# hku-mars/FAST_LIO

Measured on NVIDIA H100. Metric: scans/sec (30k-pt scan, 1M-pt map iEKF), higher is better.
Workload: dtype f32 geometry / f64 filter

## Files before the change

fast_lio_b200/csrc/filter.cu:

```cuda
#include <dlfcn.h>

#include <algorithm>
#include <chrono>
#include <cstdlib>

#include <cub/device/device_select.cuh>

#include "filter.h"
#include "gj.cuh"
#include "measure.cuh"

namespace fl {

constexpr int PSTRIDE = 96;
constexpr size_t P2P_MAIL_BYTES = sizeof(unsigned long long) * 2 * 2 * P2P_MAX_RANKS * PSTRIDE;
constexpr int SEARCH_THREADS = 256;
constexpr int SEARCH_C_THREADS = 256;
constexpr int RESID_THREADS = 256;
constexpr int MAX_LOGS = 16;

__device__ __forceinline__ void pdl_wait() { asm volatile("griddepcontrol.wait;" ::: "memory"); }
__device__ __forceinline__ void pdl_launch() { asm volatile("griddepcontrol.launch_dependents;" ::: "memory"); }

__device__ __forceinline__ int tri12(int a, int b) { return a * 12 - (a * (a - 1)) / 2 + (b - a); }
// ... 775 lines not shown
                                                                  const double* __restrict__ P, StateIn s) {
    pdl_launch();
    const int b = (int)blockIdx.x;
    state_in(ctl + b, pub + (size_t)b * BATCH_PUB_WORDS, x26 + (size_t)b * XLEN, P + (size_t)b * NDOF * NDOF, s);
}

__global__ void k_count_in(const int* __restrict__ n, int n_max, int* __restrict__ bind) {
    bind[0] = min(max(*n, 0), n_max);
    bind[1] = BIND_SCAN;
}

__device__ __forceinline__ void state_out(const FilterCtl* __restrict__ ctl, double* __restrict__ x26, double* __restrict__ P,
                                          int* __restrict__ status2) {
    const int t = threadIdx.x;
    const int e = ctl->error;
    if (e == 0) {
        for (int i = t; i < NDOF * NDOF; i += STATE_THREADS) P[i] = ctl->P[i];
        if (t < XLEN) x26[t] = ctl->x[t];
    }
    if (t == 0) { status2[0] = e == 0 ? FL_OK : (e == 2 ? FL_ERR_NCCL : FL_ERR_STATE); status2[1] = ctl->n_pass; }
}
__global__ void __launch_bounds__(STATE_THREADS) k_state_out(const FilterCtl* __restrict__ ctl, double* __restrict__ x26,
                                                             double* __restrict__ P, int* __restrict__ status2) {
    state_out(ctl, x26, P, status2);
}
__global__ void __launch_bounds__(STATE_THREADS) k_batch_state_out(const FilterCtl* __restrict__ ctl, double* __restrict__ x26,
                                                                   double* __restrict__ P, int* __restrict__ status2) {
    const int b = (int)blockIdx.x;
    state_out(ctl + b, x26 + (size_t)b * XLEN, P + (size_t)b * NDOF * NDOF, status2 + 2 * b);
}

__global__ void k_flags_clear(unsigned char* __restrict__ flag_add, unsigned char* __restrict__ flag_no, const int* __restrict__ n, int n_max) {
    const int q = blockIdx.x * blockDim.x + threadIdx.x;
    if (q < n_max && q >= *n) { flag_add[q] = 0; flag_no[q] = 0; }
}

struct NcclUniqueId { char internal[128]; };
struct NcclApi {
    void* lib = nullptr;
    int (*GetUniqueId)(NcclUniqueId*) = nullptr;
    int (*CommInitRank)(void**, int, NcclUniqueId, int) = nullptr;
    int (*AllReduce)(const void*, void*, size_t, int, int, void*, cudaStream_t) = nullptr;
    int (*CommDestroy)(void*) = nullptr;
    const char* (*GetErrorString)(int) = nullptr;
};
static NcclApi* load_nccl() {
    static NcclApi api;
    if (api.lib) return &api;
    const char* names[] = {"libnccl.so.2", "libnccl.so"};
    for (const char* nm : names) { api.lib = dlopen(nm, RTLD_NOW | RTLD_GLOBAL); if (api.lib) break; }
    if (!api.lib) { set_last_error("NCCL: cannot dlopen libnccl.so.2: %s", dlerror()); return nullptr; }
    api.GetUniqueId = (int (*)(NcclUniqueId*))dlsym(api.lib, "ncclGetUniqueId");
    api.CommInitRank = (int (*)(void**, int, NcclUniqueId, int))dlsym(api.lib, "ncclCommInitRank");
    api.AllReduce = (int (*)(const void*, void*, size_t, int, int, void*, cudaStream_t))dlsym(api.lib, "ncclAllReduce");
    api.CommDestroy = (int (*)(void*))dlsym(api.lib, "ncclCommDestroy");
    api.GetErrorString = (const char* (*)(int))dlsym(api.lib, "ncclGetErrorString");
    if (!api.GetUniqueId || !api.CommInitRank || !api.AllReduce || !api.CommDestroy) {
        set_last_error("NCCL: missing symbols in libnccl");
        api.lib = nullptr;
        return nullptr;
    }
    return &api;
}
int nccl_unique_id(void* out128) {
    NcclApi* api = load_nccl();
    if (!api) return FL_ERR_NCCL;
    NcclUniqueId id;
    int rc = api->GetUniqueId(&id);
    if (rc != 0) { set_last_error("ncclGetUniqueId failed: %d", rc); return FL_ERR_NCCL; }
    memcpy(out128, &id, 128);
    return FL_OK;
}

Filter::Filter(Map* map, int max_points) : map_(map), max_points_(max_points) {
    memset(&scan_, 0, sizeof(scan_));
    for (int i = 0; i < NDOF; i++) limit_[i] = 0.001;
}
Filter::~Filter() {
    cudaSetDevice(map_->device());
    if (comm_ && nccl_) nccl_->CommDestroy(comm_);
    for (int r = 0; r < P2P_MAX_RANKS; r++) if (peer_ptr_[r]) cudaIpcCloseMemHandle(peer_ptr_[r]);
    mailbox_.release(); p2p_.release();
    body_.release(); nearest_.release(); nearest_cnt_.release(); selected_.release(); normvec_.release(); plane_.release(); srange_.release();
    partials_.release(); red_.release(); ctl_.release(); ctl0_.release(); logs_.release(); pub_.release();
    mi_world_.release(); mi_flag_add_.release(); mi_flag_no_.release(); mi_list_add_.release(); mi_list_no_.release(); mi_tmp_.release(); mi_counts_.release();
    d_bind_.release();
    b_body_.release(); b_ctl_.release(); b_pub_.release(); b_partials_.release();
    b_nearest_.release(); b_nearest_cnt_.release(); b_selected_.release(); b_plane_.release(); b_srange_.release();
    if (h_ctl_) cudaFreeHost(h_ctl_);
    if (ev0_) cudaEventDestroy(ev0_);
    if (ev1_) cudaEventDestroy(ev1_);
}

int Filter::init() {
    FL_CUDA(cudaSetDevice(map_->device()));
    if (const char* e = getenv("FASTLIO_B200_NO_PDL")) pdl_ = !(e[0] == '1');
    if (const char* e = getenv("FASTLIO_B200_NO_MIRROR")) mirror_ = !(e[0] == '1');
    if (const char* e = getenv("FASTLIO_B200_SEARCH")) search_mode_ = atoi(e) ? 1 : 0;
    FL_CHECK(ctl_.reserve(sizeof(FilterCtl)));
    FL_CHECK(ctl0_.reserve(sizeof(FilterCtl)));
    FL_CHECK(red_.reserve(sizeof(double) * PSTRIDE));
    FL_CHECK(logs_.reserve(sizeof(PassLog) * MAX_LOGS));
    FL_CHECK(pub_.reserve(512));
    FL_CUDA(cudaMemsetAsync(pub_.ptr, 0, 512, stream()));
    FL_CUDA(cudaMallocHost(&h_ctl_, sizeof(FilterCtl)));
    memset(h_ctl_, 0, sizeof(FilterCtl));
    FL_CUDA(cudaMemsetAsync(ctl_.ptr, 0, sizeof(FilterCtl), stream()));
    FL_CUDA(cudaMemsetAsync(ctl0_.ptr, 0, sizeof(FilterCtl), stream()));
    FL_CUDA(cudaMemsetAsync(logs_.ptr, 0, sizeof(PassLog) * MAX_LOGS, stream()));
    int dev = map_->device(), occ = 0;
    FL_CUDA(cudaDeviceGetAttribute(&sms_, cudaDevAttrMultiProcessorCount, dev));
    if (const char* e = getenv("FASTLIO_B200_SEARCH_OCC")) search_occ_ = atoi(e);
    if (search_occ_ == 6) FL_CUDA(cudaOccupancyMaxActiveBlocksPerMultiprocessor(&occ, k_search<6>, SEARCH_THREADS, 0));
    else if (search_occ_ == 5) FL_CUDA(cudaOccupancyMaxActiveBlocksPerMultiprocessor(&occ, k_search<5>, SEARCH_THREADS, 0));
    else FL_CUDA(cudaOccupancyMaxActiveBlocksPerMultiprocessor(&occ, k_search<4>, SEARCH_THREADS, 0));
    search_grid_max_ = sms_ * std::max(1, occ);
    if (const char* e = getenv("FASTLIO_B200_LEGACY")) fused_ = !(e[0] == '1');
    FL_CUDA(cudaOccupancyMaxActiveBlocksPerMultiprocessor(&occ, k_update<false, 1>, UPD_THREADS, 0));
    upd_capacity_[0][0] = sms_ * std::max(1, occ);
    FL_CUDA(cudaOccupancyMaxActiveBlocksPerMultiprocessor(&occ, k_update<true, 1>, UPD_THREADS, 0));
    upd_capacity_[1][0] = sms_ * std::max(1, occ);
    FL_CUDA(cudaOccupancyMaxActiveBlocksPerMultiprocessor(&occ, k_update<false, 2>, 2 * UPD_THREADS, 0));
    upd_capacity_[0][1] = sms_ * occ;
    FL_CUDA(cudaOccupancyMaxActiveBlocksPerMultiprocessor(&occ, k_update<true, 2>, 2 * UPD_THREADS, 0));
    upd_capacity_[1][1] = sms_ * occ;
    FL_CUDA(cudaOccupancyMaxActiveBlocksPerMultiprocessor(&occ, k_update_n<false, 1>, UPD_THREADS, 0));
    upd_n_capacity_[0][0] = std::min(upd_capacity_[0][0], sms_ * std::max(1, occ));
    FL_CUDA(cudaOccupancyMaxActiveBlocksPerMultiprocessor(&occ, k_update_n<true, 1>, UPD_THREADS, 0));
    upd_n_capacity_[1][0] = std::min(upd_capacity_[1][0], sms_ * std::max(1, occ));
    FL_CUDA(cudaOccupancyMaxActiveBlocksPerMultiprocessor(&occ, k_update_n<false, 2>, 2 * UPD_THREADS, 0));
    upd_n_capacity_[0][1] = std::min(upd_capacity_[0][1], sms_ * occ);
    FL_CUDA(cudaOccupancyMaxActiveBlocksPerMultiprocessor(&occ, k_update_n<true, 2>, 2 * UPD_THREADS, 0));
    upd_n_capacity_[1][1] = std::min(upd_capacity_[1][1], sms_ * occ);
    FL_CUDA(cudaOccupancyMaxActiveBlocksPerMultiprocessor(&occ, k_update_batch<false>, UPD_THREADS, 0));
    batch_cap_[0] = sms_ * occ;
    FL_CUDA(cudaOccupancyMaxActiveBlocksPerMultiprocessor(&occ, k_update_batch<true>, UPD_THREADS, 0));
    batch_cap_[1] = sms_ * occ;
    FL_CHECK(d_bind_.reserve(2 * sizeof(int)));
    FL_CUDA(cudaMemsetAsync(d_bind_.ptr, 0, 2 * sizeof(int), stream()));
    FL_CHECK(partials_.reserve(sizeof(double) * PSTRIDE * (size_t)std::max(upd_capacity_[0][0], upd_capacity_[1][0])));
    max_resid_grid_ = sms_;
    FL_CHECK(partials_.reserve(sizeof(double) * PSTRIDE * (size_t)max_resid_grid_));
    FL_CHECK(reserve(std::max(1, max_points_)));
    return FL_OK;
}

int Filter::reserve(int nq) {
    FL_CHECK(body_.reserve(sizeof(float4) * (size_t)nq));
    FL_CHECK(nearest_.reserve(sizeof(float4) * KNN_K * (size_t)nq));
    { const size_t had = nearest_cnt_.bytes; FL_CHECK(nearest_cnt_.reserve(sizeof(int) * (size_t)nq)); if (nearest_cnt_.bytes != had) FL_CUDA(cudaMemsetAsync(nearest_cnt_.ptr, 0, nearest_cnt_.bytes, stream())); }
    FL_CHECK(selected_.reserve((size_t)nq));
    FL_CHECK(normvec_.reserve(sizeof(float4) * (size_t)nq));
    scan_.nearest = nearest_.as<float4>();
    scan_.nearest_cnt = nearest_cnt_.as<int>();
    scan_.selected = selected_.as<unsigned char>();
    scan_.normvec = normvec_.as<float4>();
    FL_CHECK(plane_.reserve(sizeof(float4) * (size_t)nq));
    scan_.plane = plane_.as<float4>();
    FL_CHECK(srange_.reserve(sizeof(double) * (size_t)nq));
    scan_.srange = srange_.as<double>();
    FL_CHECK(mi_world_.reserve(sizeof(float4) * (size_t)nq));
    FL_CHECK(mi_flag_add_.reserve((size_t)nq));
    FL_CHECK(mi_flag_no_.reserve((size_t)nq));
    FL_CHECK(mi_list_add_.reserve(sizeof(float4) * (size_t)nq));
    FL_CHECK(mi_list_no_.reserve(sizeof(float4) * (size_t)nq));
    FL_CHECK(mi_counts_.reserve(sizeof(int) * 2));
    size_t tmp = 0;
    FL_CUDA(cub::DeviceSelect::Flagged(nullptr, tmp, (const float4*)nullptr, (const unsigned char*)nullptr, (float4*)nullptr, (int*)nullptr, nq));
    FL_CHECK(mi_tmp_.reserve(tmp));
    return FL_OK;
}

int Filter::set_params(int max_iter, const double* limit23, int extrinsic_est_en) {
    if (max_iter < 1 || max_iter + 1 > MAX_LOGS) { set_last_error("set_params: max_iter must be in [1, %d]", MAX_LOGS - 1); return FL_ERR_ARG; }
    max_iter_ = max_iter;
    if (limit23) for (int i = 0; i < NDOF; i++) limit_[i] = limit23[i];
    extrinsic_est_ = extrinsic_est_en ? 1 : 0;
    return FL_OK;
}

int Filter::set_scan_device(const float4* d_body, int nq) {
    FL_CHECK(bind_scan(d_body, nq));
    if (stream_bound_) FL_CUDA(cudaMemsetAsync(d_bind_.as<int>() + 1, 0, sizeof(int), stream()));
    return FL_OK;
}
int Filter::bind_scan(const float4* d_body, int nq) {
    if (nq < 0) { set_last_error("scan: nq < 0"); return FL_ERR_ARG; }
    FL_CUDA(cudaSetDevice(map_->device()));
    FL_CHECK(reserve(std::max(1, nq)));
    scan_.body = d_body;
    scan_.Q = nq;
    if (!shard_set_) { scan_.q_begin = 0; scan_.q_end = nq; }
    dev_count_ = false;
    return FL_OK;
}

int Filter::upload_scan(const float* body_xyzi, int nq) {
    if (nq < 0 || (nq > 0 && !body_xyzi)) { set_last_error("scan: bad arguments"); return FL_ERR_ARG; }
    FL_CUDA(cudaSetDevice(map_->device()));
    FL_CHECK(reserve(std::max(1, nq)));
    if (nq > 0) FL_CUDA(cudaMemcpyAsync(body_.ptr, body_xyzi, sizeof(float4) * (size_t)nq, cudaMemcpyHostToDevice, stream()));
    return set_scan_device(body_.as<float4>(), nq);
}

int Filter::set_shard(int q_begin, int q_end) {
    if (q_begin < 0 || q_end < q_begin) { set_last_error("set_shard: bad range"); return FL_ERR_ARG; }
    scan_.q_begin = q_begin; scan_.q_end = q_end;
    shard_set_ = true;
    return FL_OK;
}

int Filter::upload_state(const double* x26, const double* P, double R, bool snapshot) {
    FL_CUDA(cudaSetDevice(map_->device()));
    FL_CUDA(cudaStreamSynchronize(stream()));
    FilterCtl& c = *h_ctl_;
    c.iter = -1; c.t = 0; c.converge = 1; c.done = 0; c.n_pass = 0; c.error = 0; c.ticket = 0; c.gen = 0;
    c.max_iter = max_iter_;
    c.host_mirror = (mirror_ && !snapshot) ? h_ctl_ : nullptr;
    c.extrinsic_est = extrinsic_est_;
    c.R = R;
    for (int i = 0; i < NDOF; i++) c.limit[i] = limit_[i];
    memcpy(c.x, x26, sizeof(double) * XLEN);
    memcpy(c.x_prop, x26, sizeof(double) * XLEN);
    memcpy(c.P, P, sizeof(double) * NDOF * NDOF);
    memcpy(c.P_prop, P, sizeof(double) * NDOF * NDOF);
    FL_CUDA(cudaMemcpyAsync(ctl_.ptr, h_ctl_, sizeof(FilterCtl), cudaMemcpyHostToDevice, stream()));
    if (snapshot) FL_CUDA(cudaMemcpyAsync(ctl0_.ptr, ctl_.ptr, sizeof(FilterCtl), cudaMemcpyDeviceToDevice, stream()));
    return FL_OK;
}

int Filter::restore_state() {
    FL_CUDA(cudaSetDevice(map_->device()));
    FL_CUDA(cudaMemcpyAsync(ctl_.ptr, ctl0_.ptr, sizeof(FilterCtl), cudaMemcpyDeviceToDevice, stream()));
    return FL_OK;
}

template <class... KArgs, class... Args>
static cudaError_t launch_pdl(void (*kernel)(KArgs...), dim3 grid, int block, cudaStream_t st, bool pdl, Args... args) {
    cudaLaunchConfig_t cfg;
    memset(&cfg, 0, sizeof(cfg));
    cfg.gridDim = grid; cfg.blockDim = dim3((unsigned)block); cfg.dynamicSmemBytes = 0; cfg.stream = st;
    cudaLaunchAttribute attr[1];
    attr[0].id = cudaLaunchAttributeProgrammaticStreamSerialization;
    attr[0].val.programmaticStreamSerializationAllowed = pdl ? 1 : 0;
    cfg.attrs = attr; cfg.numAttrs = 1;
    return cudaLaunchKernelEx(&cfg, kernel, KArgs(args)...);
}

int Filter::complete_neighbours() {
    if (neighbours_complete_ || (scan_.q_begin <= 0 && scan_.q_end >= scan_.Q)) { neighbours_complete_ = true; return FL_OK; }
    FL_CUDA(cudaSetDevice(map_->device()));
    const int keep_b = scan_.q_begin, keep_e = scan_.q_end;
    const int ranges[2][2] = {{0, keep_b}, {keep_e, scan_.Q}};
    for (int r = 0; r < 2; r++) {
        if (ranges[r][1] <= ranges[r][0]) continue;
        scan_.q_begin = ranges[r][0]; scan_.q_end = ranges[r][1];
        UpdArgs a;
        a.m = map_->view();
        if (search_mode_ == 0) a.m.dir.cap = 0;
        a.sc = scan_; a.ctl = ctl_.as<FilterCtl>(); a.partials = partials_.as<double>(); a.red_g = red_.as<double>();
        a.logs = logs_.as<PassLog>(); a.p2p = p2p_.as<P2PState>();
        a.mode = 0; a.max_passes = 1; a.search_only = 1; a.dbg = 0; a.pose_from_search = 1;
        a.pub = pub_.as<unsigned long long>(); a.nonce = ++launch_nonce_;
        const int cap = upd_capacity_[extrinsic_est_ ? 1 : 0][0];
        const int nq = scan_.q_end - scan_.q_begin;
        const int workers = std::max(1, std::min(cap - 1, (nq + UPD_THREADS - 1) / UPD_THREADS));
        cudaError_t e = launch_upd(workers, false, a, upd_pair(nq));
        if (e != cudaSuccess) { scan_.q_begin = keep_b; scan_.q_end = keep_e; set_last_error("complete_neighbours: %s", cudaGetErrorString(e)); return FL_ERR_CUDA; }
    }
    scan_.q_begin = keep_b; scan_.q_end = keep_e;
    neighbours_complete_ = true;
    return FL_OK;
}

int Filter::run_passes() {
    FL_CUDA(cudaSetDevice(map_->device()));
    if (scan_.q_end > scan_.Q) { set_last_error("shard exceeds the scan"); return FL_ERR_ARG; }
    neighbours_complete_ = false;
    launches_ = 0;
    if (fused()) {
        cudaStream_t st = stream();
        if (nranks_ > 1 && !p2p_on_) {
            for (int pass = 0; pass <= max_iter_; pass++) {
                FL_CHECK(launch_update(1, 1, 0));
                int rc = nccl_->AllReduce(red_.ptr, red_.ptr, NRED,  8,  0, comm_, st);
                if (rc != 0) { set_last_error("ncclAllReduce failed: %d", rc); return FL_ERR_NCCL; }
                FL_CHECK(launch_update(1, 3, 0));
                launches_ += 2;
            }
        } else {
            FL_CHECK(launch_update(max_iter_ + 1, nranks_ > 1 ? 2 : 0, 0));
            launches_ = 1;
        }
        FL_CUDA(cudaGetLastError());
        return FL_OK;
    }
    for (int pass = 0; pass <= max_iter_; pass++) {
        FL_CHECK(launch_search_only());
        FL_CHECK(launch_residual_only());
        launches_ += 2;
        if (nranks_ > 1 && !p2p_on_) {
            cudaStream_t st = stream();
            int rc = nccl_->AllReduce(red_.ptr, red_.ptr, NRED,  8,  0, comm_, st);
            if (rc != 0) { set_last_error("ncclAllReduce failed: %d", rc); return FL_ERR_NCCL; }
            FilterCtl* c = ctl_.as<FilterCtl>(); double* rg = red_.as<double>(); PassLog* lg = logs_.as<PassLog>();
            if (extrinsic_est_) { if (solver_) k_solve_only<true, 1><<<1, RESID_THREADS, 0, st>>>(c, rg, scan_, lg); else k_solve_only<true, 0><<<1, RESID_THREADS, 0, st>>>(c, rg, scan_, lg); }
            else { if (solver_) k_solve_only<false, 1><<<1, RESID_THREADS, 0, st>>>(c, rg, scan_, lg); else k_solve_only<false, 0><<<1, RESID_THREADS, 0, st>>>(c, rg, scan_, lg); }
            launches_++;
        }
    }
    FL_CUDA(cudaGetLastError());
    return FL_OK;
}

UpdArgs Filter::upd_args(int max_passes, int mode, int search_only) {
    UpdArgs a;
    a.m = map_->view();
    if (search_mode_ == 0) a.m.dir.cap = 0;
    a.sc = scan_; a.ctl = ctl_.as<FilterCtl>(); a.partials = partials_.as<double>(); a.red_g = red_.as<double>();
    a.logs = logs_.as<PassLog>(); a.p2p = p2p_.as<P2PState>();
    a.mode = mode; a.max_passes = max_passes; a.search_only = search_only;
    a.pub = pub_.as<unsigned long long>(); a.nonce = ++launch_nonce_;
    { const char* e = getenv("FASTLIO_B200_DBG"); a.dbg = e ? atoi(e) : 0; }
    a.pose_from_search = 0;
    return a;
}

int Filter::launch_update(int max_passes, int mode, int search_only, cudaStream_t st) {
    FL_CUDA(cudaSetDevice(map_->device()));
    const int nq = scan_.q_end - scan_.q_begin;
    const UpdArgs a = upd_args(max_passes, mode, search_only);
    const int cap = upd_capacity_[extrinsic_est_ ? 1 : 0][0];
    int workers = mode == 3 ? 0 : std::min(cap - 1, (nq + UPD_THREADS - 1) / UPD_THREADS);
    if (workers < 0) workers = 0;
    FL_CUDA(launch_upd(workers, pdl_, a, upd_pair(nq), st));
    return FL_OK;
}

int Filter::upd_pair(int nq) const {
    if (const char* e = getenv("FASTLIO_B200_PAIR")) if (e[0] == '1') return 1;
    const int tiles = (nq + UPD_THREADS - 1) / UPD_THREADS;
    return tiles >= 1 && tiles <= upd_capacity_[extrinsic_est_ ? 1 : 0][1] - 1 ? 2 : 1;
}
cudaError_t Filter::launch_upd(int workers, bool pdl, const UpdArgs& a, int pair, cudaStream_t st) {
    const int block = pair * UPD_THREADS;
    if (extrinsic_est_) return pair == 2 ? launch_pdl(k_update<true, 2>, workers + 1, block, st, pdl, a)
                                         : launch_pdl(k_update<true, 1>, workers + 1, block, st, pdl, a);
    return pair == 2 ? launch_pdl(k_update<false, 2>, workers + 1, block, st, pdl, a)
                     : launch_pdl(k_update<false, 1>, workers + 1, block, st, pdl, a);
}

int Filter::launch_search_only() {
    FL_CUDA(cudaSetDevice(map_->device()));
    const int nq = scan_.q_end - scan_.q_begin;
    if (fused()) return launch_update(1, 0, 1);
    if (search_mode_ == 1) {
        const int cgrid = std::max(1, (nq + SEARCH_C_THREADS - 1) / SEARCH_C_THREADS);
        FL_CUDA(launch_pdl(k_search_c, cgrid, SEARCH_C_THREADS, stream(), pdl_, map_->view(), scan_, (const FilterCtl*)ctl_.as<FilterCtl>()));
        return FL_OK;
    }
    const int sgrid = std::max(1, std::min(search_grid_max_, (nq * 32 + SEARCH_THREADS - 1) / SEARCH_THREADS));
    const FilterCtl* cc = ctl_.as<FilterCtl>();
    if (search_occ_ == 6) FL_CUDA(launch_pdl(k_search<6>, sgrid, SEARCH_THREADS, stream(), pdl_, map_->view(), scan_, cc));
    else if (search_occ_ == 5) FL_CUDA(launch_pdl(k_search<5>, sgrid, SEARCH_THREADS, stream(), pdl_, map_->view(), scan_, cc));
    else FL_CUDA(launch_pdl(k_search<4>, sgrid, SEARCH_THREADS, stream(), pdl_, map_->view(), scan_, cc));
    return FL_OK;
}
int Filter::launch_residual_only() {
    FL_CUDA(cudaSetDevice(map_->device()));
    const int nq = scan_.q_end - scan_.q_begin;
    resid_grid_ = std::min(max_resid_grid_ - 1, (nq + RESID_THREADS - 1) / RESID_THREADS) + 1;
    const int mode = nranks_ > 1 ? (p2p_on_ ? 2 : 1) : 0;
    P2PState* p2p = p2p_.as<P2PState>();
    FilterCtl* c = ctl_.as<FilterCtl>(); double* pp = partials_.as<double>(); double* rg = red_.as<double>(); PassLog* lg = logs_.as<PassLog>();
    cudaStream_t st = stream();
    if (extrinsic_est_) {
        if (solver_) FL_CUDA(launch_pdl(k_residual<true, 1>, resid_grid_, RESID_THREADS, st, pdl_, scan_, c, pp, rg, mode, lg, p2p));
        else FL_CUDA(launch_pdl(k_residual<true, 0>, resid_grid_, RESID_THREADS, st, pdl_, scan_, c, pp, rg, mode, lg, p2p));
    } else {
        if (solver_) FL_CUDA(launch_pdl(k_residual<false, 1>, resid_grid_, RESID_THREADS, st, pdl_, scan_, c, pp, rg, mode, lg, p2p));
        else FL_CUDA(launch_pdl(k_residual<false, 0>, resid_grid_, RESID_THREADS, st, pdl_, scan_, c, pp, rg, mode, lg, p2p));
    }
    FL_CUDA(cudaGetLastError());
    return FL_OK;
}
int Filter::sync() {
    FL_CUDA(cudaSetDevice(map_->device()));
    FL_CUDA(cudaStreamSynchronize(stream()));
    return FL_OK;
}

int Filter::download_state(double* x26, double* P, int* n_pass) {
    FL_CUDA(cudaSetDevice(map_->device()));
    FL_CUDA(cudaStreamSynchronize(stream()));
    if (!(mirror_ && h_ctl_->done)) {
        FL_CUDA(cudaMemcpyAsync(h_ctl_, ctl_.ptr, offsetof(FilterCtl, P_prop), cudaMemcpyDeviceToHost, stream()));
        FL_CUDA(cudaStreamSynchronize(stream()));
    }
    if (h_ctl_->error) {
        const int e = h_ctl_->error;
        set_last_error(e == 2 ? "update: a peer rank never delivered its sums (peer-memory exchange timed out)"
                              : (e == 3 ? "update: a block gave up waiting for the solver / the workers on the device" : "update: singular system on device"));
        return e == 2 ? FL_ERR_NCCL : FL_ERR_STATE;
    }
    if (x26) memcpy(x26, h_ctl_->x, sizeof(double) * XLEN);
    if (P) memcpy(P, h_ctl_->P, sizeof(double) * NDOF * NDOF);
    if (n_pass) *n_pass = h_ctl_->n_pass;
    return FL_OK;
}

int Filter::update(const float* body_xyzi, int nq, double* x26, double* P, double R, double* solve_time_s) {
    return update_any(body_xyzi, nullptr, nq, x26, P, R, solve_time_s);
}
int Filter::update_device(const float4* d_body, int nq, double* x26, double* P, double R, double* solve_time_s) {
    if (nq > 0 && !d_body) { set_last_error("update: null device scan"); return FL_ERR_ARG; }
    return update_any(nullptr, d_body, nq, x26, P, R, solve_time_s);
}
int Filter::update_any(const float* body_xyzi, const float4* d_body, int nq, double* x26, double* P, double R, double* solve_time_s) {
// ... 37 lines not shown
    return (int)std::min<size_t>(c, INT_MAX);
}

int Filter::device_form_scope(const char* what, bool update) const {
    if (shard_set_ || nranks_ > 1 || p2p_on_) {
        set_last_error("%s: a sharded filter (set_shard / comm_init / p2p_connect) has no device-buffer form", what);
        return FL_ERR_STATE;
    }
    if (update && !fused()) {
        set_last_error("%s: the device-buffer form runs k_update only; this filter uses %s", what,
                       solver_ != 1 ? "solver mode 0" : "the two-kernels-per-pass chain (fused 0)");
        return FL_ERR_STATE;
    }
    return FL_OK;
}

int Filter::update_on_stream(const float* d_body, int nq, double* d_x26, double* d_P, double R, int* d_status2, cudaStream_t st) {
    const int dev = map_->device();
    if (nq < 0 || (nq > 0 && !device_ptr(d_body, dev, 16)) || !device_ptr(d_x26, dev, 8) || !device_ptr(d_P, dev, 8) ||
        !device_ptr(d_status2, dev, 4)) {
        set_last_error("update_device: nq < 0, or a buffer is not device memory on device %d (scan 16-byte, x and P 8-byte, "
                       "status 4-byte aligned)", dev);
        return FL_ERR_ARG;
    }
    FL_CHECK(device_form_scope("update_device", true));
    if (nq > capacity()) {
        set_last_error("update_device: %d points exceed the filter's capacity of %d (max_points, or the largest scan so far)", nq, capacity());
        return FL_ERR_CAPACITY;
    }
    FL_CUDA(cudaSetDevice(dev));
    bool joined = false;
    FL_CHECK(map_->query_begin(st, &joined));
    FL_CHECK(bind_scan(body_.as<float4>(), nq));
    stream_bound_ = true;
    if (nq > 0) FL_CUDA(cudaMemcpyAsync(body_.ptr, d_body, sizeof(float4) * (size_t)nq, cudaMemcpyDeviceToDevice, st));
    StateIn s;
    for (int i = 0; i < NDOF; i++) s.limit[i] = limit_[i];
    s.R = R; s.max_iter = max_iter_; s.extrinsic_est = extrinsic_est_;
    k_state_in<<<1, STATE_THREADS, 0, st>>>(ctl_.as<FilterCtl>(), pub_.as<unsigned long long>(), h_ctl_, d_x26, d_P, s, d_bind_.as<int>(), nq);
    FL_CUDA(cudaGetLastError());
    neighbours_complete_ = false;
    FL_CHECK(launch_update(max_iter_ + 1, 0, 0, st));
    launches_ = 1;
    k_state_out<<<1, STATE_THREADS, 0, st>>>(ctl_.as<FilterCtl>(), d_x26, d_P, d_status2);
    return map_->query_end(st, joined);
}

int Filter::update_scan_on_stream(const float4* d_body, const int* d_n, int n_max, double* d_x26, double* d_P, double R, int* d_status2,
                                  cudaStream_t st) {
    const int dev = map_->device();
    if (!device_ptr(d_x26, dev, 8) || !device_ptr(d_P, dev, 8) || !device_ptr(d_status2, dev, 4)) {
        set_last_error("update_scan_device: a buffer is not device memory on device %d (x and P 8-byte, status 4-byte aligned)", dev);
        return FL_ERR_ARG;
    }
    FL_CHECK(device_form_scope("update_scan_device", true));
    if (n_max > capacity()) {
        set_last_error("update_scan_device: the scan's n_max of %d exceeds the filter's capacity of %d (max_points, or the largest scan so far)",
                       n_max, capacity());
        return FL_ERR_CAPACITY;
    }
    FL_CUDA(cudaSetDevice(dev));
    bool joined = false;
    FL_CHECK(map_->query_begin(st, &joined));
    FL_CHECK(bind_scan(d_body, n_max));
    dev_count_ = true;
    q_max_ = n_max;
    scan_body_ = d_body;
    stream_bound_ = true;
    k_count_in<<<1, 1, 0, st>>>(d_n, n_max, d_bind_.as<int>());
    StateIn s;
    for (int i = 0; i < NDOF; i++) s.limit[i] = limit_[i];
    s.R = R; s.max_iter = max_iter_; s.extrinsic_est = extrinsic_est_;
    k_state_in<<<1, STATE_THREADS, 0, st>>>(ctl_.as<FilterCtl>(), pub_.as<unsigned long long>(), h_ctl_, d_x26, d_P, s, nullptr, 0);
    FL_CUDA(cudaGetLastError());
    neighbours_complete_ = false;
    const int e = extrinsic_est_ ? 1 : 0;
    const int tiles = (n_max + UPD_THREADS - 1) / UPD_THREADS;
    const int pair = upd_pair(n_max) == 2 && tiles <= upd_n_capacity_[e][1] - 1 ? 2 : 1;
    const int workers = std::max(0, std::min(upd_n_capacity_[e][0] - 1, tiles));
    const UpdArgs a = upd_args(max_iter_ + 1, 0, 0);
    const int* n = d_bind_.as<int>();
    const int block = pair * UPD_THREADS;
    cudaError_t rc;
    if (e) rc = pair == 2 ? launch_pdl(k_update_n<true, 2>, workers + 1, block, st, pdl_, a, n) : launch_pdl(k_update_n<true, 1>, workers + 1, block, st, pdl_, a, n);
    else rc = pair == 2 ? launch_pdl(k_update_n<false, 2>, workers + 1, block, st, pdl_, a, n) : launch_pdl(k_update_n<false, 1>, workers + 1, block, st, pdl_, a, n);
    FL_CUDA(rc);
    launches_ = 1;
    k_state_out<<<1, STATE_THREADS, 0, st>>>(ctl_.as<FilterCtl>(), d_x26, d_P, d_status2);
    return map_->query_end(st, joined);
}

int Filter::batch_plan(int nq, int n_hyp, int* workers, int* slots, int* waves) const {
    if (nq < 0 || n_hyp < 0) { set_last_error("batch_plan: nq and n_hyp must be >= 0"); return FL_ERR_ARG; }
    const int e = extrinsic_est_ ? 1 : 0;
    const int w = std::max(0, std::min(upd_capacity_[e][0] - 1, (nq + UPD_THREADS - 1) / UPD_THREADS));
    if (w + 1 > batch_cap_[e]) {
        set_last_error("batch_plan: a hypothesis takes %d blocks, %d k_update_batch blocks are co-resident", w + 1, batch_cap_[e]);
        return FL_ERR_CAPACITY;
    }
    const int s = batch_cap_[e] / (w + 1);
    *workers = w;
    *slots = s;
    *waves = (n_hyp + s - 1) / s;
    return FL_OK;
}

int Filter::reserve_batch(int nq_max) {
    if (nq_max < 0) { set_last_error("reserve_batch: nq_max must be >= 0"); return FL_ERR_ARG; }
    if (nq_max > capacity()) {
        set_last_error("reserve_batch: %d points exceed the filter's capacity of %d (max_points, or the largest scan so far)", nq_max, capacity());
        return FL_ERR_CAPACITY;
    }
    FL_CUDA(cudaSetDevice(map_->device()));
    size_t rows = 1;
    int cap = 1;
    for (int e = 0; e < 2; e++) {
        const int wmax = std::max(0, std::min(upd_capacity_[e][0] - 1, (nq_max + UPD_THREADS - 1) / UPD_THREADS));
        for (int w = 0; w <= wmax && w + 1 <= batch_cap_[e]; w++) {
            const int nq_hi = w == wmax ? nq_max : std::min(nq_max, UPD_THREADS * w);
            rows = std::max(rows, (size_t)(batch_cap_[e] / (w + 1)) * (size_t)nq_hi);
        }
        cap = std::max(cap, batch_cap_[e]);
    }
    FL_CHECK(b_body_.reserve(sizeof(float4) * (size_t)std::max(1, nq_max)));
    FL_CHECK(b_ctl_.reserve(sizeof(FilterCtl) * (size_t)cap));
    FL_CHECK(b_pub_.reserve(sizeof(unsigned long long) * BATCH_PUB_WORDS * (size_t)cap));
    FL_CHECK(b_partials_.reserve(sizeof(double) * PSTRIDE * (size_t)cap));
    FL_CHECK(b_nearest_.reserve(sizeof(float4) * KNN_K * rows));
    FL_CHECK(b_nearest_cnt_.reserve(sizeof(int) * rows));
    FL_CHECK(b_selected_.reserve(rows));
    FL_CHECK(b_plane_.reserve(sizeof(float4) * rows));
    FL_CHECK(b_srange_.reserve(sizeof(double) * rows));
    FL_CUDA(cudaMemsetAsync(b_ctl_.ptr, 0, b_ctl_.bytes, stream()));
    FL_CUDA(cudaMemsetAsync(b_pub_.ptr, 0, b_pub_.bytes, stream()));
    FL_CUDA(cudaStreamSynchronize(stream()));
    batch_nq_max_ = std::max(batch_nq_max_, nq_max);
    return FL_OK;
}

int Filter::update_batch_on_stream(const float* d_body, int nq, int n_hyp, double* d_x26, double* d_P, double R, int* d_status2,
                                   PassLog* d_logs, cudaStream_t st) {
    const int dev = map_->device();
    if (nq < 0 || n_hyp < 0 || (nq > 0 && !device_ptr(d_body, dev, 16)) ||
        (n_hyp > 0 && (!device_ptr(d_x26, dev, 8) || !device_ptr(d_P, dev, 8) || !device_ptr(d_status2, dev, 4) ||
                       (d_logs && !device_ptr(d_logs, dev, 8))))) {
        set_last_error("update_batch_device: nq or n_hyp < 0, or a buffer is not device memory on device %d (scan 16-byte, x, P and "
                       "logs 8-byte, status 4-byte aligned)", dev);
        return FL_ERR_ARG;
    }
    FL_CHECK(device_form_scope("update_batch_device", true));
    if (batch_nq_max_ < 0) { set_last_error("update_batch_device: call fl_filter_reserve_batch first"); return FL_ERR_STATE; }
    if (nq > batch_nq_max_) {
        set_last_error("update_batch_device: %d points exceed the %d fl_filter_reserve_batch sized", nq, batch_nq_max_);
        return FL_ERR_CAPACITY;
    }
    int workers = 0, slots = 0, waves = 0;
    FL_CHECK(batch_plan(nq, n_hyp, &workers, &slots, &waves));
    if (n_hyp == 0) return FL_OK;
    FL_CUDA(cudaSetDevice(dev));
    bool joined = false;
    FL_CHECK(map_->query_begin(st, &joined));
    if (nq > 0) FL_CUDA(cudaMemcpyAsync(b_body_.ptr, d_body, sizeof(float4) * (size_t)nq, cudaMemcpyDeviceToDevice, st));
    ScanView sc;
    memset(&sc, 0, sizeof(sc));
    sc.body = b_body_.as<float4>();
    sc.nearest = b_nearest_.as<float4>(); sc.nearest_cnt = b_nearest_cnt_.as<int>(); sc.selected = b_selected_.as<unsigned char>();
    sc.plane = b_plane_.as<float4>(); sc.srange = b_srange_.as<double>();
// ... 260 lines not shown
```

fast_lio_b200/csrc/filter.h:

```cpp
#pragma once
#include "lie.cuh"
#include "map.h"

namespace fl {

struct PassLog {
    int searched, valid, effct, converged;
    double res_sum;
    double HtH[144];
    double Hth[12];
    double x_after[XLEN];
};

struct FilterCtl {
    int iter;
    int t;
    int converge;
    int done;
    int n_pass;
    int max_iter;
    int extrinsic_est;
    int error;
    int ticket;
    int gen;
// ... 44 lines not shown
    void set_solver(int mode) { solver_ = mode; }

    int update(const float* body_xyzi, int nq, double* x26, double* P, double R, double* solve_time_s);
    int update_device(const float4* d_body, int nq, double* x26, double* P, double R, double* solve_time_s);
    int upload_scan(const float* body_xyzi, int nq);
    int set_scan_device(const float4* d_body, int nq);
    int upload_state(const double* x26, const double* P, double R, bool snapshot = true);
    int restore_state();
    int run_passes();
    int launch_search_only();
    int launch_residual_only();
    int download_state(double* x26, double* P, int* n_pass);
    int sync();
    int update_on_stream(const float* d_body, int nq, double* d_x26, double* d_P, double R, int* d_status2, cudaStream_t st);
    int get_nearest_on_stream(float* d_pts, int* d_cnt, int nq, cudaStream_t st);
    int get_selected_on_stream(unsigned char* d_out, int nq, cudaStream_t st);
    int update_scan_on_stream(const float4* d_body, const int* d_n, int n_max, double* d_x26, double* d_P, double R, int* d_status2, cudaStream_t st);
    int capacity() const;
    int reserve_batch(int nq_max);
    int batch_plan(int nq, int n_hyp, int* workers, int* slots, int* waves) const;
    int update_batch_on_stream(const float* d_body, int nq, int n_hyp, double* d_x26, double* d_P, double R, int* d_status2,
                               PassLog* d_logs, cudaStream_t st);

    int map_incremental(double filter_size_map_min, int ekf_inited, int* n_to_add, int* n_no_downsample, int* added);
    int map_incremental_on_stream(double filter_size_map_min, int ekf_inited, int* d_out4, cudaStream_t st);
    int get_nearest(float* out_pts, int* out_cnt, int nq);
    int complete_neighbours();
    int get_selected(unsigned char* out, int nq);
    int get_pass_logs(PassLog* out, int cap, int* n);
    int comm_init(int nranks, int rank, const void* nccl_unique_id_128);
    int set_shard(int q_begin, int q_end);
    int p2p_local_handle(void* out64);
    int p2p_connect(int nranks, int rank, const void* handles64);
    int p2p_barrier();

    void set_fused(bool on) { fused_ = on; }
    bool fused() const { return fused_ && solver_ == 1; }
    int gpu_launches() const { return launches_; }
    const long long* host_ns() const { return host_ns_; }
    const float4* nearest_device() const { return scan_.nearest; }
    const ScanView& scan() const { return scan_; }
    cudaStream_t stream() const { return map_->stream(); }
    Map* map() const { return map_; }
    const FilterCtl* ctl_device() const { return ctl_.as<FilterCtl>(); }

private:
    int reserve(int nq);
    int update_any(const float* body_xyzi, const float4* d_body, int nq, double* x26, double* P, double R, double* solve_time_s);
    Map* map_;
    int max_points_;
    int max_iter_ = 4;
    double limit_[NDOF];
    int extrinsic_est_ = 0;
    int solver_ = 1;
    bool mirror_ = true;
    bool pdl_ = true;
    int search_occ_ = 5;
    int search_mode_ = 1;
    ScanView scan_;
    DeviceBuffer srange_;
    DeviceBuffer body_, nearest_, nearest_cnt_, selected_, normvec_, plane_, partials_, red_, ctl_, ctl0_, logs_;
    DeviceBuffer mi_world_, mi_flag_add_, mi_flag_no_, mi_list_add_, mi_list_no_, mi_tmp_, mi_counts_;
    FilterCtl* h_ctl_ = nullptr;
    cudaEvent_t ev0_ = nullptr, ev1_ = nullptr;
    int sms_ = 0, search_grid_max_ = 0, max_resid_grid_ = 0, resid_grid_ = 1;
    bool fused_ = true;
    DeviceBuffer pub_;
    unsigned launch_nonce_ = 0;
    int upd_capacity_[2][2] = {{0, 0}, {0, 0}};
    int launch_update(int max_passes, int mode, int search_only) { return launch_update(max_passes, mode, search_only, stream()); }
    int launch_update(int max_passes, int mode, int search_only, cudaStream_t st);
    int upd_pair(int nq) const;
    cudaError_t launch_upd(int workers, bool pdl, const UpdArgs& a, int pair) { return launch_upd(workers, pdl, a, pair, stream()); }
    cudaError_t launch_upd(int workers, bool pdl, const UpdArgs& a, int pair, cudaStream_t st);
    int device_form_scope(const char* what, bool update) const;
    UpdArgs upd_args(int max_passes, int mode, int search_only);
    int bind_scan(const float4* d_body, int nq);
    bool dev_count_ = false;
    int q_max_ = 0;
    const float4* scan_body_ = nullptr;
    bool stream_bound_ = false;
    DeviceBuffer d_bind_;
    int upd_n_capacity_[2][2] = {{0, 0}, {0, 0}};
    int read_binding();
    int batch_cap_[2] = {0, 0};
    int batch_nq_max_ = -1;
    DeviceBuffer b_body_, b_ctl_, b_pub_, b_partials_, b_nearest_, b_nearest_cnt_, b_selected_, b_plane_, b_srange_;
    int launches_ = 0;
    long long host_ns_[4] = {0, 0, 0, 0};
    bool shard_set_ = false;
    bool neighbours_complete_ = true;
    NcclApi* nccl_ = nullptr;
    void* comm_ = nullptr;
    int nranks_ = 1, rank_ = 0;
    DeviceBuffer mailbox_, p2p_;
    void* peer_ptr_[P2P_MAX_RANKS] = {nullptr};
    bool p2p_on_ = false;
};

}
```

fast_lio_b200/csrc/update.cuh:

```cuda
#pragma once

namespace fl {

constexpr int UPD_THREADS = 256;
constexpr int UPD_WARPS = UPD_THREADS / 32;

struct UpdArgs {
    MapView m;
    ScanView sc;
    FilterCtl* ctl;
    double* partials;
    double* red_g;
    PassLog* logs;
    P2PState* p2p;
    unsigned long long* pub;
    unsigned nonce;
    int mode;
    int max_passes;
    int search_only;
    int dbg;
    int pose_from_search;
};

struct SolverSm {
// ... 634 lines not shown
#pragma unroll
                for (int j = 0; j < 3; j++) Wk.wred[warp][lane + 32 * j] = acc[j];
            }
            __syncthreads();
            if (tid < PSTRIDE) {
                double v = 0.0;
#pragma unroll
                for (int w = 0; w < UPD_WARPS; w++) v += Wk.wred[w][tid];
                __stcg(&a.partials[(size_t)wb * PSTRIDE + tid], v);
            }
            __syncthreads();
            if (tid == 0) asm volatile("red.release.gpu.global.add.s32 [%0], 1;" ::"l"(&ctl->ticket) : "memory");
            if (a.mode == 1) return;
        }
        return;
    }
    if (a.search_only) return;
    if (tid >= UPD_THREADS) return;
    SolverSm& S = *reinterpret_cast<SolverSm*>(smem_raw);
    sol_load(S, ctl);
    int p = 0;
    for (; p < a.max_passes && !S.done; p++) {
        if (tid == 0) ctl->prof[0] = clock64();
        if (S.converge && tid < XLEN) ctl->x_search[tid] = S.x[tid];
        if (a.mode != 1) sol_prepare(S);
        if (tid == 0) ctl->prof[8] = clock64();
        if (a.mode != 3) {
            if (tid == 0) {
                const long long t0 = clock64();
                while (ld_acquire(&ctl->ticket) < nwork * (p + 1)) {
                    if (clock64() - t0 > SPIN_LIMIT) { S.late = 2; break; }
                }
            }
            sol_sync();
            if (tid == 0) ctl->prof[9] = clock64();
            sol_reduce(S, a.partials, nwork);
            if (a.mode == 1) {
                if (tid < NRED) a.red_g[tid] = S.red[tid];
                if (tid == 0) ctl->ticket = 0;
                return;
            }
        } else {
            if (tid < PSTRIDE) S.red[tid] = tid < NRED ? a.red_g[tid] : 0.0;
            sol_sync();
            sol_expand(S);
        }
        if (a.mode == 2) { sol_exchange(S, a.p2p); sol_expand(S); }
        if (tid == 0) ctl->prof[1] = clock64();
        sol_pass<EXTR>(S, ctl, a.logs, a.pub, pub_tag(a.nonce, p + 1));
        if (tid == 0) ctl->prof[7] = clock64();
    }
    if (tid == 0) { ctl->error = S.error | ctl->error; ctl->ticket = 0; }
    sol_sync();
    mirror_copy(ctl, UPD_THREADS);
}

template <bool EXTR, int PAIR>
__global__ void __launch_bounds__(UPD_THREADS * PAIR, 3 - PAIR) k_update(UpdArgs a) {
    update_body<EXTR, PAIR>(a, a.sc.q_end);
}

template <bool EXTR, int PAIR>
__global__ void __launch_bounds__(UPD_THREADS * PAIR, 3 - PAIR) k_update_n(UpdArgs a, const int* __restrict__ n) {
    update_body<EXTR, PAIR>(a, min(*n, a.sc.q_end));
}

constexpr int BATCH_PUB_WORDS = 32;
template <bool EXTR>
__global__ void __launch_bounds__(UPD_THREADS, 2) k_update_batch(UpdArgs a, int log_stride) {
    const int s = (int)blockIdx.y;
    const size_t rows = (size_t)s * (size_t)a.sc.Q;
    a.ctl += s;
    a.partials += (size_t)s * (gridDim.x - 1) * PSTRIDE;
    a.pub += (size_t)s * BATCH_PUB_WORDS;
    if (a.logs) a.logs += (size_t)s * log_stride;
    a.sc.nearest += rows * KNN_K;
    a.sc.nearest_cnt += rows;
    a.sc.selected += rows;
    a.sc.plane += rows;
    a.sc.srange += rows;
    update_body<EXTR, 1>(a, a.sc.q_end);
}

}
```

Measured before the change: 11790.

## Add wave update kernel with tagged per-worker row publication and smem point cache

Adds a new persistent iEKF update kernel (k_update_wave and k_update_n_wave) for the paired-block case. Each worker block writes its reduced HᵀH/Hᵀz row into a dedicated tagged slot in a rows buffer, and the solver block gathers and sums these slots by polling the tags. This replaces the previous shared-partials reduction path. Each worker also caches its points' body coordinates, plane, range and selection flag in dynamic shared memory across passes, which avoids reloading them from global memory. The trade-off is more spin-polling traffic, extra dynamic shared memory that may cut occupancy, and an epoch protocol that has to stay consistent across launches.

```diff
diff --git a/fast_lio_b200/csrc/filter.cu b/fast_lio_b200/csrc/filter.cu
--- a/fast_lio_b200/csrc/filter.cu
+++ b/fast_lio_b200/csrc/filter.cu
@@ -881,7 +881,7 @@
     for (int r = 0; r < P2P_MAX_RANKS; r++) if (peer_ptr_[r]) cudaIpcCloseMemHandle(peer_ptr_[r]);
     mailbox_.release(); p2p_.release();
     body_.release(); nearest_.release(); nearest_cnt_.release(); selected_.release(); normvec_.release(); plane_.release(); srange_.release();
-    partials_.release(); red_.release(); ctl_.release(); ctl0_.release(); logs_.release(); pub_.release();
+    partials_.release(); red_.release(); ctl_.release(); ctl0_.release(); logs_.release(); pub_.release(); rows_.release();
     mi_world_.release(); mi_flag_add_.release(); mi_flag_no_.release(); mi_list_add_.release(); mi_list_no_.release(); mi_tmp_.release(); mi_counts_.release();
     d_bind_.release();
     b_body_.release(); b_ctl_.release(); b_pub_.release(); b_partials_.release();
@@ -935,6 +935,23 @@
     batch_cap_[0] = sms_ * occ;
     FL_CUDA(cudaOccupancyMaxActiveBlocksPerMultiprocessor(&occ, k_update_batch<true>, UPD_THREADS, 0));
     batch_cap_[1] = sms_ * occ;
+    FL_CUDA(cudaFuncSetAttribute(k_update_wave<false>, cudaFuncAttributeMaxDynamicSharedMemorySize, (int)sizeof(WavePoint)));
+    FL_CUDA(cudaFuncSetAttribute(k_update_wave<true>, cudaFuncAttributeMaxDynamicSharedMemorySize, (int)sizeof(WavePoint)));
+    FL_CUDA(cudaFuncSetAttribute(k_update_n_wave<false>, cudaFuncAttributeMaxDynamicSharedMemorySize, (int)sizeof(WavePoint)));
+    FL_CUDA(cudaFuncSetAttribute(k_update_n_wave<true>, cudaFuncAttributeMaxDynamicSharedMemorySize, (int)sizeof(WavePoint)));
+    FL_CUDA(cudaOccupancyMaxActiveBlocksPerMultiprocessor(&occ, k_update_wave<false>, 2 * UPD_THREADS, sizeof(WavePoint)));
+    wave_capacity_[0] = sms_ * occ;
+    FL_CUDA(cudaOccupancyMaxActiveBlocksPerMultiprocessor(&occ, k_update_wave<true>, 2 * UPD_THREADS, sizeof(WavePoint)));
+    wave_capacity_[1] = sms_ * occ;
+    FL_CUDA(cudaOccupancyMaxActiveBlocksPerMultiprocessor(&occ, k_update_n_wave<false>, 2 * UPD_THREADS, sizeof(WavePoint)));
+    wave_n_capacity_[0] = std::min(wave_capacity_[0], sms_ * occ);
+    FL_CUDA(cudaOccupancyMaxActiveBlocksPerMultiprocessor(&occ, k_update_n_wave<true>, 2 * UPD_THREADS, sizeof(WavePoint)));
+    wave_n_capacity_[1] = std::min(wave_capacity_[1], sms_ * occ);
+    {
+        const size_t bytes = sizeof(unsigned long long) * 2 * PSTRIDE * (size_t)std::max(1, std::max(wave_capacity_[0], wave_capacity_[1]));
+        FL_CHECK(rows_.reserve(bytes));
+        FL_CUDA(cudaMemsetAsync(rows_.ptr, 0, bytes, stream()));
+    }
     FL_CHECK(d_bind_.reserve(2 * sizeof(int)));
     FL_CUDA(cudaMemsetAsync(d_bind_.ptr, 0, 2 * sizeof(int), stream()));
     FL_CHECK(partials_.reserve(sizeof(double) * PSTRIDE * (size_t)std::max(upd_capacity_[0][0], upd_capacity_[1][0])));
@@ -1035,15 +1052,19 @@
 }
 
 template <class... KArgs, class... Args>
-static cudaError_t launch_pdl(void (*kernel)(KArgs...), dim3 grid, int block, cudaStream_t st, bool pdl, Args... args) {
+static cudaError_t launch_pdl_smem(void (*kernel)(KArgs...), dim3 grid, int block, size_t smem, cudaStream_t st, bool pdl, Args... args) {
     cudaLaunchConfig_t cfg;
     memset(&cfg, 0, sizeof(cfg));
-    cfg.gridDim = grid; cfg.blockDim = dim3((unsigned)block); cfg.dynamicSmemBytes = 0; cfg.stream = st;
+    cfg.gridDim = grid; cfg.blockDim = dim3((unsigned)block); cfg.dynamicSmemBytes = smem; cfg.stream = st;
     cudaLaunchAttribute attr[1];
     attr[0].id = cudaLaunchAttributeProgrammaticStreamSerialization;
     attr[0].val.programmaticStreamSerializationAllowed = pdl ? 1 : 0;
     cfg.attrs = attr; cfg.numAttrs = 1;
     return cudaLaunchKernelEx(&cfg, kernel, KArgs(args)...);
+}
+template <class... KArgs, class... Args>
+static cudaError_t launch_pdl(void (*kernel)(KArgs...), dim3 grid, int block, cudaStream_t st, bool pdl, Args... args) {
+    return launch_pdl_smem(kernel, grid, block, 0, st, pdl, args...);
 }
 
 int Filter::complete_neighbours() {
@@ -1132,7 +1153,14 @@
     const int cap = upd_capacity_[extrinsic_est_ ? 1 : 0][0];
     int workers = mode == 3 ? 0 : std::min(cap - 1, (nq + UPD_THREADS - 1) / UPD_THREADS);
     if (workers < 0) workers = 0;
-    FL_CUDA(launch_upd(workers, pdl_, a, upd_pair(nq), st));
+    const int pair = upd_pair(nq);
+    if (use_wave(workers, pair, mode)) {
+        unsigned long long* rows = rows_.as<unsigned long long>();
+        FL_CUDA(extrinsic_est_ ? launch_pdl_smem(k_update_wave<true>, workers + 1, 2 * UPD_THREADS, sizeof(WavePoint), st, pdl_, a, rows)
+                               : launch_pdl_smem(k_update_wave<false>, workers + 1, 2 * UPD_THREADS, sizeof(WavePoint), st, pdl_, a, rows));
+        return FL_OK;
+    }
+    FL_CUDA(launch_upd(workers, pdl_, a, pair, st));
     return FL_OK;
 }
 
@@ -1336,7 +1364,11 @@
     const int* n = d_bind_.as<int>();
     const int block = pair * UPD_THREADS;
     cudaError_t rc;
-    if (e) rc = pair == 2 ? launch_pdl(k_update_n<true, 2>, workers + 1, block, st, pdl_, a, n) : launch_pdl(k_update_n<true, 1>, workers + 1, block, st, pdl_, a, n);
+    if (pair == 2 && workers + 1 <= wave_n_capacity_[e]) {
+        unsigned long long* rows = rows_.as<unsigned long long>();
+        rc = e ? launch_pdl_smem(k_update_n_wave<true>, workers + 1, block, sizeof(WavePoint), st, pdl_, a, n, rows)
+               : launch_pdl_smem(k_update_n_wave<false>, workers + 1, block, sizeof(WavePoint), st, pdl_, a, n, rows);
+    } else if (e) rc = pair == 2 ? launch_pdl(k_update_n<true, 2>, workers + 1, block, st, pdl_, a, n) : launch_pdl(k_update_n<true, 1>, workers + 1, block, st, pdl_, a, n);
     else rc = pair == 2 ? launch_pdl(k_update_n<false, 2>, workers + 1, block, st, pdl_, a, n) : launch_pdl(k_update_n<false, 1>, workers + 1, block, st, pdl_, a, n);
     FL_CUDA(rc);
     launches_ = 1;
diff --git a/fast_lio_b200/csrc/filter.h b/fast_lio_b200/csrc/filter.h
--- a/fast_lio_b200/csrc/filter.h
+++ b/fast_lio_b200/csrc/filter.h
@@ -150,6 +150,9 @@
     bool stream_bound_ = false;
     DeviceBuffer d_bind_;
     int upd_n_capacity_[2][2] = {{0, 0}, {0, 0}};
+    int wave_capacity_[2] = {0, 0}, wave_n_capacity_[2] = {0, 0};
+    DeviceBuffer rows_;
+    bool use_wave(int workers, int pair, int mode) const { return mode == 0 && pair == 2 && workers + 1 <= wave_capacity_[extrinsic_est_ ? 1 : 0]; }
     int read_binding();
     int batch_cap_[2] = {0, 0};
     int batch_nq_max_ = -1;
diff --git a/fast_lio_b200/csrc/update.cuh b/fast_lio_b200/csrc/update.cuh
--- a/fast_lio_b200/csrc/update.cuh
+++ b/fast_lio_b200/csrc/update.cuh
@@ -740,4 +740,275 @@
     update_body<EXTR, 1>(a, a.sc.q_end);
 }
 
-}
+struct WavePoint {
+    float4 body[UPD_THREADS];
+    float4 plane[UPD_THREADS];
+    double srange[UPD_THREADS];
+    unsigned char sel[UPD_THREADS];
+};
+constexpr int WAVE_EPOCH = 32;
+__device__ __forceinline__ unsigned row_tag(unsigned epoch, int pass) { return pub_tag(epoch, pass + 1); }
+__device__ __forceinline__ unsigned long long globaltimer() {
+    unsigned long long t;
+    asm volatile("mov.u64 %0, %%globaltimer;" : "=l"(t));
+    return t;
+}
+__device__ __forceinline__ ulonglong2 row_load(const unsigned long long* p) {
+    ulonglong2 v;
+    asm volatile("ld.relaxed.gpu.global.v2.u64 {%0, %1}, [%2];" : "=l"(v.x), "=l"(v.y) : "l"(p) : "memory");
+    return v;
+}
+__device__ __forceinline__ bool row_current(ulonglong2 v, unsigned tag) { return (unsigned)(v.x >> 32) == tag && (unsigned)(v.y >> 32) == tag; }
+__device__ __forceinline__ double row_value(ulonglong2 v) { return __longlong_as_double((long long)((v.y << 32) | (v.x & 0xffffffffull))); }
+
+template <bool EXTR>
+__device__ __forceinline__ bool measure_wave(const MapView& m, const ScanView& sc, int q, bool active, const PoseS& s, bool searched,
+                                             bool search_only, WalkPool& walks, int& phase, double* stage, WavePoint& pt, double* h,
+                                             double& z, float& absres) {
+    const int i = threadIdx.x & (UPD_THREADS - 1);
+    float4 pb = make_float4(0.f, 0.f, 0.f, 0.f);
+    float wx = 0.f, wy = 0.f, wz = 0.f;
+    D3 p_this = d3(0.0, 0.0, 0.0);
+    if (active) {
+        pb = pt.body[i];
+        p_this = body_to_world(s, pb, wx, wy, wz);
+    }
+    bool sel = false;
+    float pabcd[4] = {0.f, 0.f, 0.f, 0.f};
+    if (searched) {
+        TBest kb;
+        knn_block_pair(m, active, wx, wy, wz, kb, walks, phase, stage);
+        if (threadIdx.x >= UPD_THREADS) return false;
+        if (active) {
+            float4 p[KNN_K];
+            const int cnt = knn_fetch(m, kb, p);
+#pragma unroll
+            for (int j = 0; j < KNN_K; j++) sc.nearest[(size_t)q * KNN_K + j] = p[j];
+            sc.nearest_cnt[q] = cnt;
+            sel = knn_gate(cnt, kb.d[KNN_K - 1]);
+            if (search_only) { sc.selected[q] = sel ? 1 : 0; return false; }
+            if (sel) {
+                float pn[KNN_K][3];
+#pragma unroll
+                for (int j = 0; j < KNN_K; j++) { pn[j][0] = p[j].x; pn[j][1] = p[j].y; pn[j][2] = p[j].z; }
+                sel = esti_plane_dev(pabcd, pn, 0.1f);
+                if (sel) { const float4 pl = make_float4(pabcd[0], pabcd[1], pabcd[2], pabcd[3]); sc.plane[q] = pl; pt.plane[i] = pl; }
+            }
+        }
+    } else if (active) {
+        sel = pt.sel[i] != 0;
+        if (sel) { const float4 pl = pt.plane[i]; pabcd[0] = pl.x; pabcd[1] = pl.y; pabcd[2] = pl.z; pabcd[3] = pl.w; }
+    }
+    bool contrib = false;
+    if (active && sel) {
+        const float pd2 = plane_residual(pabcd, wx, wy, wz);
+        const double srange = pt.srange[i];
+        if (searched) sc.srange[q] = srange;
+        float score;
+        if (score_gate(pd2, srange, score)) {
+            contrib = true;
+            absres = fabsf(pd2);
+            jacobian_row_at<EXTR>(s, pb, p_this, make_float4(pabcd[0], pabcd[1], pabcd[2], pd2), h, z);
+        }
+    }
+    if (active) { sc.selected[q] = contrib ? 1 : 0; pt.sel[i] = contrib ? 1 : 0; }
+    return contrib;
+}
+
+constexpr int GATHER_ROWS = 8;
+__device__ void sol_gather(SolverSm& S, FilterCtl* ctl, const unsigned long long* __restrict__ rows, int nwork, unsigned tag) {
+    const int tid = threadIdx.x, lane = tid & 31, warp = tid >> 5;
+    double a0 = 0.0, a1 = 0.0, a2 = 0.0;
+    bool late = false;
+    const long long t0 = clock64();
+    for (int b = warp; b < nwork; b += GATHER_ROWS * UPD_WARPS) {
+        const unsigned long long* base = rows + (size_t)b * PSTRIDE * 2 + 2 * lane;
+        ulonglong2 v[GATHER_ROWS][3];
+#pragma unroll
+        for (int k = 0; k < GATHER_ROWS; k++) {
+#pragma unroll
+            for (int j = 0; j < 3; j++) v[k][j] = make_ulonglong2(0ull, 0ull);
+            if (b + k * UPD_WARPS < nwork) {
+#pragma unroll
+                for (int j = 0; j < 3; j++) v[k][j] = row_load(base + (size_t)k * UPD_WARPS * PSTRIDE * 2 + 64 * j);
+            }
+        }
+        while (true) {
+            bool stale = false;
+#pragma unroll
+            for (int k = 0; k < GATHER_ROWS; k++) {
+#pragma unroll
+                for (int j = 0; j < 3; j++) stale |= b + k * UPD_WARPS < nwork && !row_current(v[k][j], tag);
+            }
+            if (!stale) break;
+            if (clock64() - t0 > SPIN_LIMIT) { late = true; break; }
+#pragma unroll
+            for (int k = 0; k < GATHER_ROWS; k++) {
+#pragma unroll
+                for (int j = 0; j < 3; j++) {
+                    if (b + k * UPD_WARPS < nwork && !row_current(v[k][j], tag)) v[k][j] = row_load(base + (size_t)k * UPD_WARPS * PSTRIDE * 2 + 64 * j);
+                }
+            }
+        }
+#pragma unroll
+        for (int k = 0; k < GATHER_ROWS; k++) {
+            if (b + k * UPD_WARPS < nwork) { a0 += row_value(v[k][0]); a1 += row_value(v[k][1]); a2 += row_value(v[k][2]); }
+        }
+        if (late) break;
+    }
+    S.wred[warp][lane] = a0; S.wred[warp][lane + 32] = a1; S.wred[warp][lane + 64] = a2;
+    if (late) S.late = 2;
+    sol_sync();
+    if (tid == 0) ctl->prof[9] = clock64();
+    if (tid < PSTRIDE) {
+        double v = 0.0;
+#pragma unroll
+        for (int w = 0; w < UPD_WARPS; w++) v += S.wred[w][tid];
+        S.red[tid] = v;
+        if (tid < 78) {
+            int a = 0, rem = tid;
+            while (rem >= 12 - a) { rem -= 12 - a; a++; }
+            const int b = a + rem;
+            S.HTH[a * 12 + b] = v; S.HTH[b * 12 + a] = v;
+        }
+    }
+    sol_sync();
+    if (tid == 128) ctl->prof[11] = (long long)globaltimer();
+}
+
+template <bool EXTR>
+__device__ __forceinline__ void update_wave_body(const UpdArgs& a, unsigned long long* __restrict__ rows, const int q1) {
+    static_assert(sizeof(PairXch) <= sizeof(double) * WorkerSm<EXTR>::STAGE, "the partner's list fits the owner warp's stage slice");
+    __shared__ __align__(16) unsigned char smem_raw[sizeof(SolverSm) > sizeof(WorkerSm<EXTR>) ? sizeof(SolverSm) : sizeof(WorkerSm<EXTR>)];
+    extern __shared__ __align__(16) unsigned char wave_dyn[];
+    __shared__ volatile int solver_ended;
+    FilterCtl* ctl = a.ctl;
+    const int tid = threadIdx.x, lane = tid & 31, warp = tid >> 5;
+    const int nwork = (int)gridDim.x - 1;
+    pdl_wait();
+    pdl_launch();
+    const unsigned epoch = (unsigned)__ldcg(a.pub + WAVE_EPOCH) + 1u;
+    if (blockIdx.x > 0) {
+        WorkerSm<EXTR>& Wk = *reinterpret_cast<WorkerSm<EXTR>*>(smem_raw);
+        WavePoint& pt = *reinterpret_cast<WavePoint*>(wave_dyn);
+        const int wb = (int)blockIdx.x - 1;
+        const int i = tid & (UPD_THREADS - 1), q = a.sc.q_begin + wb * UPD_THREADS + i;
+        const bool active = q < q1, owner = tid < UPD_THREADS;
+        if (tid == 0) { Wk.abort = 0; Wk.walks.n[0] = Wk.walks.n[1] = 0; }
+        int walk_phase = 0;
+        double* stage = Wk.stage[warp & (UPD_WARPS - 1)];
+        for (int p = 0; p < a.max_passes; p++) {
+            PoseS s;
+            bool searched;
+            if (p == 0) {
+                const bool done = __ldcg(&ctl->done) != 0;
+                searched = __ldcg(&ctl->converge) != 0 || a.search_only;
+                s = load_pose(a.pose_from_search ? ctl->x_search : ctl->x);
+                if (owner && active) {
+                    const float4 pb = __ldg(&a.sc.body[q]);
+                    pt.body[i] = pb;
+                    pt.srange[i] = sqrt(norm3(d3(pb.x, pb.y, pb.z)));
+                    if (!searched) {
+                        pt.sel[i] = a.sc.selected[q];
+                        if (pt.sel[i]) { pt.plane[i] = a.sc.plane[q]; pt.srange[i] = a.sc.srange[q]; }
+                    }
+                }
+                __syncthreads();
+                if (done && !a.search_only) return;
+            } else {
+                const unsigned tag = pub_tag(a.nonce, p);
+                if (warp == 0 && lane < PUB_WORDS) {
+                    unsigned long long w = pub_load(a.pub + lane);
+                    const long long t0 = clock64();
+                    while ((unsigned)(w >> 32) != tag) {
+                        if (clock64() - t0 > SPIN_LIMIT) { Wk.abort = 1; atomicExch(&ctl->error, 3); break; }
+                        w = pub_load(a.pub + lane);
+                    }
+                    if (lane < 28) Wk.pose_bits[lane] = (unsigned)w; else Wk.flags = (unsigned)w;
+                }
+                __syncthreads();
+                if (Wk.abort) return;
+                if (Wk.flags & 2u) {
+                    if (tid == 0) atomicMax(reinterpret_cast<unsigned long long*>(&ctl->prof[3]), globaltimer());
+                    return;
+                }
+                searched = (Wk.flags & 1u) != 0;
+                double x14[14];
+#pragma unroll
+                for (int k = 0; k < 14; k++) x14[k] = __longlong_as_double((long long)(((unsigned long long)Wk.pose_bits[2 * k + 1] << 32) | Wk.pose_bits[2 * k]));
+                s.pos = d3(x14[X_POS], x14[X_POS + 1], x14[X_POS + 2]);
+                s.rot.x = x14[X_ROT]; s.rot.y = x14[X_ROT + 1]; s.rot.z = x14[X_ROT + 2]; s.rot.w = x14[X_ROT + 3];
+                s.offR.x = x14[X_OFFR]; s.offR.y = x14[X_OFFR + 1]; s.offR.z = x14[X_OFFR + 2]; s.offR.w = x14[X_OFFR + 3];
+                s.offT = d3(x14[X_OFFT], x14[X_OFFT + 1], x14[X_OFFT + 2]);
+            }
+            double acc[3] = {0.0, 0.0, 0.0};
+            double h[12]; double z = 0.0; float ar = 0.f;
+            bool contrib = false;
+            if (owner || searched)
+                contrib = measure_wave<EXTR>(a.m, a.sc, q, active, s, searched, a.search_only != 0, Wk.walks, walk_phase, stage, pt, h, z, ar);
+            if (owner && !a.search_only) warp_accumulate<EXTR>(contrib, h, z, ar, acc, lane, stage);
+            if (a.search_only) return;
+            if (owner) {
+#pragma unroll
+                for (int j = 0; j < 3; j++) Wk.wred[warp][lane + 32 * j] = acc[j];
+            }
+            __syncthreads();
+            if (tid < PSTRIDE) {
+                double v = 0.0;
+#pragma unroll
+                for (int w = 0; w < UPD_WARPS; w++) v += Wk.wred[w][tid];
+                const unsigned long long bits = (unsigned long long)__double_as_longlong(v);
+                unsigned long long* dst = rows + ((size_t)wb * PSTRIDE + tid) * 2;
+                const unsigned tag = row_tag(epoch, p);
+                pub_store(dst, tag, (unsigned)bits);
+                pub_store(dst + 1, tag, (unsigned)(bits >> 32));
+            }
+        }
+        return;
+    }
+    if (a.search_only) return;
+    if (tid == 0) solver_ended = 0;
+    __syncthreads();
+    if (tid >= UPD_THREADS) {
+        if (tid == UPD_THREADS) {
+            for (int p = 1; p <= a.max_passes; p++) {
+                const unsigned tag = pub_tag(a.nonce, p);
+                unsigned long long w;
+                while ((unsigned)((w = pub_load(a.pub + 28)) >> 32) != tag) if (solver_ended) return;
+                ctl->prof[2] = (long long)globaltimer();
+                if (w & 2u) return;
+            }
+        }
+        return;
+    }
+    SolverSm& S = *reinterpret_cast<SolverSm*>(smem_raw);
+    sol_load(S, ctl);
+    for (int p = 0; p < a.max_passes && !S.done; p++) {
+        if (tid == 0) ctl->prof[0] = clock64();
+        if (S.converge && tid < XLEN) ctl->x_search[tid] = S.x[tid];
+        sol_prepare(S);
+        if (tid == 0) ctl->prof[8] = clock64();
+        sol_gather(S, ctl, rows, nwork, row_tag(epoch, p));
+        if (tid == 0) ctl->prof[1] = clock64();
+        sol_pass<EXTR>(S, ctl, a.logs, a.pub, pub_tag(a.nonce, p + 1));
+        if (tid == 0) ctl->prof[7] = clock64();
+    }
+    if (tid == 0) {
+        ctl->error = S.error | ctl->error; ctl->ticket = 0;
+        a.pub[WAVE_EPOCH] = epoch;
+        solver_ended = 1;
+    }
+    sol_sync();
+    mirror_copy(ctl, UPD_THREADS);
+}
+
+template <bool EXTR>
+__global__ void __launch_bounds__(2 * UPD_THREADS, 1) k_update_wave(UpdArgs a, unsigned long long* rows) {
+    update_wave_body<EXTR>(a, rows, a.sc.q_end);
+}
+template <bool EXTR>
+__global__ void __launch_bounds__(2 * UPD_THREADS, 1) k_update_n_wave(UpdArgs a, const int* __restrict__ n, unsigned long long* rows) {
+    update_wave_body<EXTR>(a, rows, min(*n, a.sc.q_end));
+}
+
+}
```

Result: faster. 12340 (median of 6 runs) (+4.7%).
